# Iheckzza/FeatureMatching

Measured on AMD Instinct MI355X. Metric: image-pairs/sec at 640x480 (coarse corr + dual-softmax mutual-NN + fine window refinement), higher is better.
Workload: dtype i8 screening + f32 exact; 1 GPU; 640x480 pair, C=256 @1/8 (L=S=4800), Cf=64 @1/2, 5x5 fine window, 'peaky' descriptors; launch=hipGraph replay, concurrent_streams=4, fine_maps_layout=nchw

## Files before the change

featurematching_amd/csrc/api.hip:

```cpp
#include <math.h>
#include <stdlib.h>

#include "fm_debug.h"
#include "fm_internal.h"

namespace fm {

int g_unit_cert = 0;

int choose_splits(int N, int panels, int tiles, int target) {
  const int wg = N * panels;
#ifdef FM_TUNE_ENV
  if (const char* e = getenv("FM_TARGET_WGS")) target = atoi(e) > 0 ? atoi(e) : 256;
#endif
  int s = target / (wg > 0 ? wg : 1);
  if (s < 1) s = 1;
  const int smax = tiles / 2 > 0 ? tiles / 2 : 1;
  if (s > smax) s = smax;
  if (s > 32) s = 32;
  return s;
}

static int choose_screen_chunks(int N, int Lp, int nunits, int* units_per_chunk, bool alone) {
  const long nrb = (long)N * (Lp / 32);
// ... 10 lines not shown
  C = padded_channels(C);
  w.N = N; w.L = L; w.S = S; w.C = C; w.slots = slots;
  w.Lp = round_up(L, kPanelRows);
  w.Sp = round_up(S, kTileCols);
  w.panels = w.Lp / kPanelRows;
  w.tiles = w.Sp / kTileCols;
  w.splits = choose_splits(N, w.panels, w.tiles);
  {
    int target = N * w.panels >= kMaxPassSlots ? 10 * kMaxPassSlots : (alone ? kMaxPassSlots : kMaxPassTarget);
    if (target == kMaxPassTarget && w.tiles / choose_splits(N, w.panels, w.tiles, kMaxPassTarget) >= 32) target = kMaxPassSlots;
    w.splits0 = choose_splits(N, w.panels, w.tiles, target);
    w.top2 = N * w.panels < kMaxPassSlots && w.tiles / choose_splits(N, w.panels, w.tiles, kMaxPassTarget) < 32;
  }
#ifdef FM_TUNE_ENV
  if (const char* e = getenv("FM_TARGET_WGS0")) w.splits0 = choose_splits(N, w.panels, w.tiles, atoi(e) > 0 ? atoi(e) : kMaxPassTarget);
#endif
  w.splits_s = choose_screen_chunks(N, w.Lp, w.Sp / 32, &w.units_s, alone);
  const size_t rows = (size_t)N * w.Lp, cols = (size_t)N * w.Sp;
  const size_t nblk = (rows * slots + 255) / 256;
  size_t o = 0;
  auto take = [&](auto& r, size_t count) { r.at = o; o = align256(o + r.bytes(count)); };
  auto since = [&](size_t at) { return Span{at, o - at}; };
  take(w.cand.count, rows);
  take(w.ccand.count, cols);
  take(w.cand_b.count, rows);
  take(w.ccand_b.count, cols);
  take(w.dense_cnt, N);
  w.counters[0] = since(w.cand.count.at);
  take(w.cell0, rows);
  take(w.cell1, cols);
  take(w.ties0, kTieCap + 1);
  take(w.ties1, kTieCap + 1);
  w.reassign[0] = since(w.cell0.at);
  take(w.rowmax_u, rows);
  take(w.colmax_u, cols);
  take(w.blocktot, nblk);
  w.reassign[1] = since(w.blocktot.at);
  take(w.scalars, 1);
  w.reassign[2] = Span{w.scalars.at, sizeof(Scalars::flags)};
  w.counters[1] = Span{w.scalars.at, sizeof(Scalars)};
  w.prep_zero = since(w.cand.count.at);
  take(w.q0, rows * C); take(w.q1, cols * C);
  take(w.sigimg, (size_t)N * 2);
  take(w.imgstat, (size_t)N * 8);
  take(w.l1_0, rows); take(w.l1_1, cols);
  take(w.bstat0, rows / 32); take(w.bstat1, cols / 32);
  take(w.emarg, N);
  take(w.nmr, rows); take(w.nmc, cols);
  take(w.umax, rows / 32 * (cols / N / 32));
  take(w.cand.idx, rows * slots); take(w.cand.x, rows * slots);
  take(w.ccand.idx, cols * slots); take(w.ccand.x, cols * slots);
  take(w.thr_r, rows); take(w.thr_c, cols);
  take(w.wmaxb, rows / 32); take(w.cmaxu, cols / 32);
  take(w.tmin_r, rows / 32); take(w.tmin_c, cols / 32);
  take(w.umax2, rows / 32 * (cols / N / 32));
  take(w.upos, rows / 32 * (cols / N / 32));
  w.common_total = o;
  take(w.hi0, rows * C); take(w.lo0, rows * C);
  take(w.hi1, cols * C); take(w.lo1, cols * C);
  take(w.f16inv, N);
  take(w.rowB, rows * w.splits); take(w.colB, cols * w.panels);
  take(w.rsum, rows); take(w.csum, cols);
  take(w.nmr2, rows); take(w.nmc2, cols);
  take(w.cand_b.idx, rows * slots); take(w.cand_b.x, rows * slots);
  take(w.ccand_b.idx, cols * slots); take(w.ccand_b.x, cols * slots);
  w.total = o;
  return w;
}

}

using namespace fm;

extern "C" int fm_version(void) { return FM_VERSION; }

extern "C" const char* fm_strerror(int s) {
  switch (s) {
    case FM_OK: return "ok";
    case FM_E_NULL: return "required pointer is NULL";
    case FM_E_SHAPE: return "inconsistent or non-positive shape";
    case FM_E_UNSUPPORTED: return "unsupported configuration (C % 4 == 0 and C <= 256, Cf = 64, W in {5,7}, thr in (0,1))";
    case FM_E_WORKSPACE: return "workspace too small or not 256-byte aligned";
    case FM_E_CAPACITY: return "more matches than the output capacity";
    case FM_E_CANDIDATES: return "a coarse row or column exceeded its candidate slots (FM_MODE_EXACT_SCREENING, then more cand_slots)";
    case FM_E_RANGE: return "descriptor not finite or |x| >= 32768, or similarities of several thousand (screening margin >= 2^60)";
    case FM_E_DENSE: return "flat similarity in a sample: call again with FM_MODE_DENSE";
    case FM_E_INTERNAL: return "assignment kernel: bounded wait for predecessor workgroups ran out; call again";
    case FM_E_STEP: return "int8 screening step too small for a descriptor outside the sampled rows: call again with FM_MODE_EXACT_STEP";
    default: return s > 0 ? hipGetErrorString((hipError_t)s) : "unknown fmatch status";
  }
}

extern "C" int fm_default_cand_slots(float thr) {
  if (!(thr > 0.f)) return 64;
  int need = (int)ceilf(1.0f / thr) + 3;
  int s = 8;
  while (s < need && s < 64) s <<= 1;
  return s;
}

static float inv_ct_of(int C, float temperature) { return 1.0f / ((float)C * temperature); }

static bool valid_slots(int s) { return s >= 4 && s <= 64 && (s & (s - 1)) == 0; }

constexpr int kKnownModes = FM_MODE_DENSE | FM_MODE_EXACT_SCREENING | FM_MODE_NO_CELL_MAPS | FM_MODE_EXACT_STEP | FM_MODE_STATS |
                            FM_MODE_FLAT | FM_MODE_ALONE;

// ... 56 lines not shown
  return FM_OK;
}

extern "C" int fm_coarse_workspace_bytes(int N, int L, int S, int C, int cand_slots, size_t* bytes) {
  return fm_coarse_workspace_bytes_mode(N, L, S, C, cand_slots, FM_MODE_DENSE | FM_MODE_EXACT_SCREENING, 1, bytes);
}

extern "C" int fm_debug_coarse_layout(int N, int L, int S, int C, int cand_slots, int64_t* out, int n_out) {
  if (!out) return FM_E_NULL;
  if (n_out < 40) return FM_E_SHAPE;
  CoarseWs w;
  if (const int bad = checked_layout(true, N, L, S, C, cand_slots, &w)) return bad;
  const auto at = [](const auto& r) { return (int64_t)r.at; };
  const int64_t v[41] = {w.N, w.L, w.S, w.C, w.Lp, w.Sp, w.panels, w.tiles, w.splits, w.slots,
                         at(w.cand.count), at(w.ccand.count), at(w.scalars), at(w.blocktot), at(w.hi0), at(w.lo0),
                         at(w.hi1), at(w.lo1), at(w.q0), at(w.q1), at(w.sigimg), at(w.l1_0), at(w.nmr), at(w.nmr),
                         at(w.rowB), at(w.colB), at(w.nmr), at(w.nmc), at(w.rsum), at(w.csum), at(w.cand.idx),
                         at(w.cand.x), at(w.ccand.idx), at(w.umax), at(w.dense_cnt), at(w.rowmax_u), at(w.colmax_u),
                         w.splits_s, w.units_s, (int64_t)w.total, (int64_t)w.common_total};
  for (int i = 0; i < 40; ++i) out[i] = v[i];
  if (n_out > 40) out[40] = v[40];
  return FM_OK;
}

template <int K>
static hipError_t clear_spans(char* base, const Span (&spans)[K], hipStream_t st) {
  for (const Span& s : spans) {
    const hipError_t e = hipMemsetAsync(base + s.at, 0, s.bytes, st);
    if (e != hipSuccess) return e;
  }
  return hipSuccess;
}

static int coarse_match_impl(const CoarseCall& c, const MapCopyJob* job, bool resume) {
  if (!c.feat0 || !c.feat1 || !c.workspace || !c.d_count) return FM_E_NULL;
  if (c.in_dtype != FM_F32 && c.in_dtype != FM_F16 && c.in_dtype != FM_BF16) return FM_E_UNSUPPORTED;
  if (c.cap > 0 && (!c.b_ids || !c.i_ids || !c.j_ids || !c.mkpts0_c || !c.mkpts1_c || !c.mconf)) return FM_E_NULL;
  if (c.cap < 0 || c.L != c.h0c * c.w0c || c.S != c.h1c * c.w1c) return FM_E_SHAPE;
  if (const int bad = check_coarse_shape(c.N, c.L, c.S, c.C, c.cand_slots)) return bad;
  if (!(c.thr > 0.f) || !(c.thr < 1.f) || !(c.temperature > 0.f)) return FM_E_UNSUPPORTED;
  if (c.mode & ~kKnownModes) return FM_E_UNSUPPORTED;
  const CoarsePlan p = plan_coarse(c.mode, c.conf_matrix != nullptr, c.cand_slots);
  const CoarseWs w = coarse_layout(c.N, c.L, c.S, c.C, c.cand_slots, p.alone);
  if (c.workspace_bytes < p.workspace_bytes(w) || ((uintptr_t)c.workspace & 255)) return FM_E_WORKSPACE;
  char* base = (char*)c.workspace;
  hipStream_t st = (hipStream_t)c.stream;
  const float inv_ct = inv_ct_of(c.C, c.temperature);
  const float thr_list = fminf(c.thr, p.list_cap);
#define FM_TRY(call) do { const hipError_t e_ = (call); if (e_ != hipSuccess) return (int)e_; } while (0)
  if (!resume) {
    FM_TRY(launch_prep(c.feat0, c.feat1, c.in_dtype, c.C, w, base, p.exact_step, p.flat, st));
    FM_TRY(launch_max_i8(w, base, unit_cert_on(w, !p.dense), st));
    if (p.flat) FM_TRY(launch_stab(w, base, inv_ct, c.thr, p.allow_dead, st));
    else FM_TRY(launch_screen(c.feat0, c.feat1, c.in_dtype, c.C, w, base, inv_ct, c.thr, p.dense, p.allow_dead, st));
  } else {
    FM_TRY(clear_spans(base, w.reassign, st));
  }
  if (p.prep_f16) FM_TRY(launch_prep_f16(c.feat0, c.feat1, c.in_dtype, c.C, w, base, p.f16_force, st));
  if (p.dense) FM_TRY(launch_dense(w, base, inv_ct, thr_list, st));
  if (p.reduce) FM_TRY(launch_reduce(w, base, inv_ct, st));
  if (p.rescreen) FM_TRY(launch_dense(w, base, inv_ct, thr_list, st, nullptr, 1));
  if (p.exact_lists) FM_TRY(launch_exact_lists(w, base, inv_ct, c.feat0, c.feat1, c.in_dtype, c.C, st));
  if (p.conf) {
    FM_TRY(launch_dense(w, base, inv_ct, c.thr, st, c.conf_matrix));
    FM_TRY(launch_conf_patch(w, base, inv_ct, c.conf_matrix, st));
  }
#undef FM_TRY
  return (int)launch_select(w, base, c, inv_ct, p.select(), job);
}

extern "C" int fm_coarse_match(const float* feat0, const float* feat1, int N, int L, int S, int C, int h0c, int w0c,
                               int h1c, int w1c, float temperature, float thr, int border_rm, float scale_px,
                               const float* scale0, const float* scale1, void* workspace, size_t workspace_bytes,
                               int cand_slots, int mode, int64_t* b_ids, int64_t* i_ids, int64_t* j_ids,
                               float* mkpts0_c, float* mkpts1_c, float* mconf, int cap, int32_t* d_count,
                               float* conf_matrix, void* stream) {
  const CoarseCall c{feat0, feat1, FM_F32, N, L, S, C, h0c, w0c, h1c, w1c, temperature, thr, border_rm, scale_px, scale0, scale1,
                     workspace, workspace_bytes, cand_slots, mode, b_ids, i_ids, j_ids, mkpts0_c, mkpts1_c, mconf, cap,
                     d_count, conf_matrix, stream};
  return coarse_match_impl(c, nullptr, false);
}

extern "C" int fm_coarse_match_dtype(const void* feat0, const void* feat1, int in_dtype, int N, int L, int S, int C,
                                     int h0c, int w0c, int h1c, int w1c, float temperature, float thr, int border_rm,
                                     float scale_px, const float* scale0, const float* scale1, void* workspace,
                                     size_t workspace_bytes, int cand_slots, int mode, int64_t* b_ids,
                                     int64_t* i_ids, int64_t* j_ids, float* mkpts0_c, float* mkpts1_c, float* mconf,
                                     int cap, int32_t* d_count, float* conf_matrix, void* stream) {
  const CoarseCall c{feat0, feat1, in_dtype, N, L, S, C, h0c, w0c, h1c, w1c, temperature, thr, border_rm, scale_px, scale0,
                     scale1, workspace, workspace_bytes, cand_slots, mode, b_ids, i_ids, j_ids, mkpts0_c, mkpts1_c, mconf, cap,
                     d_count, conf_matrix, stream};
  return coarse_match_impl(c, nullptr, false);
}

extern "C" int fm_coarse_match_maps(const void* feat0, const void* feat1, int in_dtype, int N, int L, int S, int C,
                                    int h0c, int w0c, int h1c, int w1c, float temperature, float thr, int border_rm,
                                    float scale_px, const float* scale0, const float* scale1, void* workspace,
                                    size_t workspace_bytes, int cand_slots, int mode, int64_t* b_ids,
                                    int64_t* i_ids, int64_t* j_ids, float* mkpts0_c, float* mkpts1_c, float* mconf,
                                    int cap, int32_t* d_count, float* conf_matrix, const float* feat_f1, int Nf, int Cf,
                                    int Hf1, int Wf1, void* scratch1, void* stream) {
  if (!feat_f1 || !scratch1) return FM_E_NULL;
  if (Nf <= 0 || Hf1 <= 0 || Wf1 <= 0) return FM_E_SHAPE;
  if (Cf != 64) return FM_E_UNSUPPORTED;
  if (((uintptr_t)scratch1 & 15) || ((uintptr_t)feat_f1 & 15)) return FM_E_WORKSPACE;
  const MapCopyJob job{feat_f1, (float*)scratch1, Nf, Hf1, Wf1};
  const CoarseCall c{feat0, feat1, in_dtype, N, L, S, C, h0c, w0c, h1c, w1c, temperature, thr, border_rm, scale_px, scale0,
// ... 75 lines not shown
  }
  *m_out = m;
  if (info_out) *info_out = info;
  if (hint_io && (st == FM_OK || st == FM_E_CAPACITY)) {
    int learnt = cur & kAutoDataModes;
    if (full_stats) learnt &= ~FM_MODE_EXACT_SCREENING | (mode & FM_MODE_EXACT_SCREENING);
    if ((learnt & FM_MODE_DENSE) && !full_stats) {
      if (info & FM_DEV_ALL_DENSE) learnt |= FM_MODE_FLAT; else learnt &= ~FM_MODE_FLAT;
    }
    *hint_io = learnt | (slots != slots_start ? slots << 8 : 0) | (slots << 16) | (attempts << 24);
  }
  return st;
}

extern "C" int fm_coarse_cell_maps(void* workspace, int N, int L, int S, int C, int cand_slots, int32_t** cell0,
                                   int* pitch0, int32_t** ties0, int32_t** cell1, int* pitch1, int32_t** ties1) {
  CoarseWs w;
  if (const int bad = checked_layout(workspace && cell0 && cell1 && pitch0 && pitch1 && ties0 && ties1, N, L, S, C,
                                     cand_slots, &w))
    return bad;
  *cell0 = w.cell0.in(workspace); *pitch0 = w.Lp; *ties0 = w.ties0.in(workspace);
  *cell1 = w.cell1.in(workspace); *pitch1 = w.Sp; *ties1 = w.ties1.in(workspace);
  return FM_OK;
}

extern "C" int fm_coarse_softmax_stats(void* workspace, int N, int L, int S, int C, int cand_slots, const float** nm_r,
                                       const float** sum_r, int* pitch_r, const float** nm_c, const float** sum_c,
                                       int* pitch_c) {
  CoarseWs w;
  if (const int bad = checked_layout(workspace && nm_r && sum_r && pitch_r && nm_c && sum_c && pitch_c, N, L, S, C,
                                     cand_slots, &w))
    return bad;
  *nm_r = w.nmr.in(workspace); *sum_r = w.rsum.in(workspace); *pitch_r = w.Lp;
  *nm_c = w.nmc.in(workspace); *sum_c = w.csum.in(workspace); *pitch_c = w.Sp;
  return FM_OK;
}

extern "C" int fm_debug_launch_corr(void* workspace, int N, int L, int S, int C, int cand_slots, float temperature,
                                    float thr, int mode, void* stream) {
  CoarseWs w;
  if (const int bad = checked_layout(workspace, N, L, S, C, cand_slots, &w)) return bad;
  if (mode < 0 || mode > 2) return FM_E_UNSUPPORTED;
  hipStream_t st = (hipStream_t)stream;
  if (mode == 0) return (int)launch_max_i8(w, (char*)workspace, unit_cert_on(w), st);
  if (mode == 1) return (int)launch_dense(w, (char*)workspace, inv_ct_of(C, temperature), thr, st);
  return (int)launch_dense(w, (char*)workspace, inv_ct_of(C, temperature), thr, st, nullptr, 1);
}

extern "C" int fm_debug_launch_screen(void* workspace, const float* feat0, const float* feat1, int N, int L, int S,
                                          int C, int cand_slots, float temperature, float thr, void* stream) {
  CoarseWs w;
  if (const int bad = checked_layout(workspace && feat0 && feat1, N, L, S, C, cand_slots, &w)) return bad;
  return (int)launch_screen(feat0, feat1, FM_F32, C, w, (char*)workspace, inv_ct_of(C, temperature), thr, 1, 1,
                                (hipStream_t)stream);
}

extern "C" int fm_debug_launch_prep(void* workspace, const float* feat0, const float* feat1, int N, int L, int S, int C,
                                    int cand_slots, void* stream) {
  CoarseWs w;
  if (const int bad = checked_layout(workspace && feat0 && feat1, N, L, S, C, cand_slots, &w)) return bad;
  return (int)launch_prep(feat0, feat1, FM_F32, C, w, (char*)workspace, 0, 0, (hipStream_t)stream);
}

extern "C" int fm_debug_launch_prep_f16(void* workspace, const float* feat0, const float* feat1, int N, int L, int S,
                                        int C, int cand_slots, int force, void* stream) {
  CoarseWs w;
  if (const int bad = checked_layout(workspace && feat0 && feat1, N, L, S, C, cand_slots, &w)) return bad;
  return (int)launch_prep_f16(feat0, feat1, FM_F32, C, w, (char*)workspace, force, (hipStream_t)stream);
}

extern "C" int fm_debug_launch_flat(void* workspace, const float* feat0, const float* feat1, int N, int L, int S, int C,
                                    int cand_slots, float temperature, float thr, int which, void* stream) {
  CoarseWs w;
  if (const int bad = checked_layout(workspace && feat0 && feat1, N, L, S, C, cand_slots, &w)) return bad;
  if (which < 0 || which > 1) return FM_E_UNSUPPORTED;
  if (which == 0) return (int)launch_prep(feat0, feat1, FM_F32, C, w, (char*)workspace, 0, 1, (hipStream_t)stream);
  return (int)launch_stab(w, (char*)workspace, inv_ct_of(C, temperature), thr, 1, (hipStream_t)stream);
}

extern "C" int fm_debug_reset_counters(void* workspace, int N, int L, int S, int C, int cand_slots, void* stream) {
  CoarseWs w;
  if (const int bad = checked_layout(workspace, N, L, S, C, cand_slots, &w)) return bad;
  return (int)clear_spans((char*)workspace, w.counters, (hipStream_t)stream);
}

extern "C" int fm_debug_unit_cert(int mode) {
  const int prev = g_unit_cert;
  if (mode >= 0 && mode <= 2) g_unit_cert = mode;
  return prev;
}

extern "C" int fm_debug_unit_cert_layout(int N, int L, int S, int C, int cand_slots, int64_t* out, int n_out) {
  if (!out) return FM_E_NULL;
  if (n_out < 9) return FM_E_SHAPE;
  CoarseWs w;
  if (const int bad = checked_layout(true, N, L, S, C, cand_slots, &w)) return bad;
  const int64_t v[9] = {(int64_t)w.umax.at, (int64_t)w.umax2.at, (int64_t)w.upos.at, (int64_t)w.thr_r.at, (int64_t)w.thr_c.at,
                        (int64_t)w.tmin_r.at, (int64_t)w.tmin_c.at, (int64_t)(w.scalars.at + offsetof(Scalars, cert_units)), w.top2};
  for (int i = 0; i < 9; ++i) out[i] = v[i];
  return FM_OK;
}

extern "C" int fm_read_count(const int32_t* d_count, int cap, int32_t* m_out, void* stream) {
  return fm_read_count_info(d_count, cap, m_out, nullptr, stream);
}

extern "C" int fm_read_count_info(const int32_t* d_count, int cap, int32_t* m_out, int32_t* info_out, void* stream) {
  if (!d_count || !m_out) return FM_E_NULL;
  int32_t h[2] = {0, 0};
  hipStream_t st = (hipStream_t)stream;
  hipError_t e = hipMemcpyAsync(h, d_count, sizeof(h), hipMemcpyDeviceToHost, st);
  if (e != hipSuccess) return (int)e;
  e = hipStreamSynchronize(st);
  if (e != hipSuccess) return (int)e;
  *m_out = h[0];
  if (info_out) *info_out = h[1];
  if (h[1] & FM_DEV_INTERNAL) return FM_E_INTERNAL;
  if (h[1] & FM_DEV_RANGE) return FM_E_RANGE;
  if (h[1] & FM_DEV_STEP) return FM_E_STEP;
  if (h[1] & FM_DEV_DENSE) return FM_E_DENSE;
  if (h[1] & FM_DEV_CANDIDATES) return FM_E_CANDIDATES;
  if (h[1] & FM_DEV_CAPACITY) return FM_E_CAPACITY;
  if (h[0] > cap) return FM_E_CAPACITY;
  return FM_OK;
}
```

featurematching_amd/csrc/coarse_screen.hip:

```cpp
#include <stdlib.h>
#include <string.h>

#include <type_traits>

#include "fm_device.h"
#include "fm_wave_device.h"

namespace fm {

constexpr int kMaxExact = 24;

struct ScreenArgs {
  const signed char* q0; const signed char* q1;
  const void* src0; const void* src1; int c_in, in_dtype;
  const unsigned* rowmax_u; const unsigned* colmax_u;
  const float* sigimg;
  const float* imgstat;
  const float* l1_0; const float* l1_1;
  const float4* bstat0; const float4* bstat1;
  const float* umax;
  float* nmr; float* nmc; float* emarg;
  int* dense_cnt; Scalars* scal;
  int* rcount; int* rlist_j; float* rlist_x;
  int* ccount; int* clist_i; float* clist_x;
  int L, S, Lp, Sp, slots, dense_enabled;
  int allow_dead;
  float k, lt, inv_ct, cpad;
};

__device__ __forceinline__ int sig_threshold(float nm, float emu, float inv_kss) {
  const float t = floorf((-kSkipLog2 - emu - nm) * inv_kss) - 1.f;
  return (int)fminf(fmaxf(t, -1.0e9f), 1.0e9f);
}

__global__ __launch_bounds__(256) void k_stab(ScreenArgs a, float* f16inv) {
  const int side = blockIdx.z, b = blockIdx.y;
  const int len = side ? a.S : a.L, lenp = side ? a.Sp : a.Lp;
  const int idx = blockIdx.x * 256 + threadIdx.x;
  const float sig0 = a.sigimg[b * 2], sig1 = a.sigimg[b * 2 + 1];
  const float* ist = a.imgstat + (long)b * 8;
  const float l1A_max = ist[0], clipA = ist[1], infA = ist[2], l1B_max = ist[3], clipB = ist[4], infB = ist[5];
  const float ss = sig0 * sig1;
  if (blockIdx.x == 0 && side == 0 && threadIdx.x == 0) {
    const float emarg = margin_log2(q8_margin_raw(sig0, l1A_max, clipA, sig1, l1B_max, clipB, a.cpad), a.inv_ct);
    a.emarg[b] = emarg;
    const bool clipped = clipA > 0.f || clipB > 0.f;
    const float sc0 = f16_plane_scale(127.f * sig0), sc1 = f16_plane_scale(127.f * sig1);
    f16inv[b] = (1.0f / sc0) * (1.0f / sc1);
    if (!(l1A_max < INFINITY) || !(l1B_max < INFINITY)) atomicOr(&a.scal->flags, (unsigned)FM_DEV_RANGE);
    else if (!(emarg < 60.f)) atomicOr(&a.scal->flags, (unsigned)(clipped ? FM_DEV_STEP : FM_DEV_RANGE));
    else if (!(infA * sc0 < 65504.f) || !(infB * sc1 < 65504.f)) atomicOr(&a.scal->flags, (unsigned)FM_DEV_STEP);
    a.dense_cnt[b] = 1;
    a.scal->dense_units = 1;
  }
  if (idx >= lenp) return;
  const long g = (long)b * lenp + idx;
  float nm = -INFINITY;
  if (idx < len) {
    const float ln2 = 0.69314718f;
    const float l1 = (side ? a.l1_1 : a.l1_0)[g];
    const unsigned mx = (side ? a.colmax_u : a.rowmax_u)[g];
    const bool dead = a.allow_dead && 2.002f * l1 * (side ? infA : infB) * a.inv_ct + 1e-3f <
                                          (a.lt + __builtin_log2f((float)(side ? a.L : a.S))) * ln2;
    const float mraw = side ? q8_margin_raw(sig0, l1A_max, clipA, sig1, l1, clipB, a.cpad)
                            : q8_margin_raw(sig0, l1, clipA, sig1, l1B_max, clipB, a.cpad);
    nm = dead ? -INFINITY : neg_stabiliser_log2(ss * q_decode(mx), mraw, a.inv_ct);
  }
  (side ? a.nmc : a.nmr)[g] = nm;
}

struct RowsExtra {
  int* thr_r; int* thr_c; float* wmaxb; float* cmaxu;
  int* tmin_r; int* tmin_c;
  const int* umax2; const int* upos;
  int look;
  int count_cert;
  int nchunks, chunk_units, items;
};

__global__ __launch_bounds__(256) void k_thresh(ScreenArgs a, RowsExtra x) {
  const int side = blockIdx.z, b = blockIdx.y;
  const int len = side ? a.S : a.L, lenp = side ? a.Sp : a.Lp;
  const int idx = blockIdx.x * 256 + threadIdx.x;
  const int lane = threadIdx.x & 63;
  const float sig0 = a.sigimg[b * 2], sig1 = a.sigimg[b * 2 + 1];
  const float* ist = a.imgstat + (long)b * 8;
  const float l1A_max = ist[0], clipA = ist[1], infA = ist[2], l1B_max = ist[3], clipB = ist[4], infB = ist[5];
  const float ss = sig0 * sig1;
  const float kss = a.k * ss;
  const bool screen_ok = kss > 1e-30f && kss < 1e30f;
  const float inv_kss = screen_ok ? 1.0f / kss : 0.f;
  if (blockIdx.x == 0 && side == 0 && threadIdx.x == 0) {
    const float emarg = margin_log2(q8_margin_raw(sig0, l1A_max, clipA, sig1, l1B_max, clipB, a.cpad), a.inv_ct);
    a.emarg[b] = emarg;
    const bool clipped = clipA > 0.f || clipB > 0.f;
    const float emarg0 = margin_log2(q8_margin_raw(sig0, l1A_max, 0.f, sig1, l1B_max, 0.f, a.cpad), a.inv_ct);
    if (!(l1A_max < INFINITY) || !(l1B_max < INFINITY)) atomicOr(&a.scal->flags, (unsigned)FM_DEV_RANGE);
    else if (!(emarg < 60.f)) atomicOr(&a.scal->flags, (unsigned)(clipped ? FM_DEV_STEP : FM_DEV_RANGE));
    else if (clipped && emarg > 2.0f * emarg0 + 1.0f) atomicOr(&a.scal->flags, (unsigned)FM_DEV_STEP);
  }
  if (idx >= lenp) return;
  const long g = (long)b * lenp + idx;
  const int blk = idx >> 5;
  const int nblk = lenp / 32;
  float nm = -INFINITY;
  float emu = 0.f;
  if (idx < len) {
    const float ln2 = 0.69314718f;
    const float l1 = (side ? a.l1_1 : a.l1_0)[g];
    const unsigned mx = (side ? a.colmax_u : a.rowmax_u)[g];
    const float bl1 = (side ? a.bstat1 : a.bstat0)[(long)b * nblk + blk].x;
    const bool dead = a.allow_dead && 2.002f * l1 * (side ? infA : infB) * a.inv_ct + 1e-3f <
                                          (a.lt + __builtin_log2f((float)(side ? a.L : a.S))) * ln2;
    const float mraw = side ? q8_margin_raw(sig0, l1A_max, clipA, sig1, l1, clipB, a.cpad)
                            : q8_margin_raw(sig0, l1, clipA, sig1, l1B_max, clipB, a.cpad);
    nm = dead ? -INFINITY : neg_stabiliser_log2(ss * q_decode(mx), mraw, a.inv_ct);
    emu = margin_log2(side ? q8_margin_raw(sig0, l1A_max, clipA, sig1, bl1, clipB, a.cpad)
                           : q8_margin_raw(sig0, bl1, clipA, sig1, l1B_max, clipB, a.cpad), a.inv_ct);
  }
  (side ? a.nmc : a.nmr)[g] = nm;
  const int thr = idx < len ? sig_threshold(nm, emu, inv_kss) : 0x3fffffff;
  (side ? x.thr_c : x.thr_r)[g] = thr;
  const float bm = half_all<OpMax>(nm);
  const int tm = half_all<OpMin>(thr);
  if ((lane & 31) == 0) {
    (side ? x.cmaxu : x.wmaxb)[(long)b * nblk + blk] = bm;
    (side ? x.tmin_c : x.tmin_r)[(long)b * nblk + blk] = tm;
  }
}

template <int C>
__global__ __launch_bounds__(256, 3) void k_screen_rows(ScreenArgs a, RowsExtra x) {
  constexpr int KS8 = C / 32;
  constexpr int LIST = 256;
  const int tid = threadIdx.x;
  const int lane = tid & 63;
  const int wv = __builtin_amdgcn_readfirstlane(tid >> 6);
  const int r = lane & 31, h = lane >> 5;
  __shared__ int s_list[4][LIST];

  const int nrb = a.Lp / 32, nunits = a.Sp / 32;
  const int item = xcd_contiguous(blockIdx.x, gridDim.x) * 4 + wv;
  if (item >= x.items) return;
  const int per_sample = nrb * x.nchunks;
  const int b = item / per_sample;
  int kk = item - b * per_sample;
  const int chunk = kk / nrb;
  const int rb = kk - chunk * nrb;
  const int wrow0 = rb * 32;
  if (wrow0 >= a.L) return;
  const int u0 = chunk * x.chunk_units;
  const int U = min(x.chunk_units, nunits - u0);

  const float sig0 = a.sigimg[b * 2], sig1 = a.sigimg[b * 2 + 1];
  const float* ist = a.imgstat + (long)b * 8;
  const float clipA = ist[1], clipB = ist[4];
  const float bl1A = a.bstat0[(long)b * nrb + rb].x;
  const float wmax = x.wmaxb[(long)b * nrb + rb];
  const int ul_c = min(lane, U - 1);
  const float um = a.umax[((long)b * nrb + rb) * nunits + u0 + ul_c];
  const float cm = x.cmaxu[(long)b * nunits + u0 + ul_c];
  const float bl1B = a.bstat1[(long)b * nunits + u0 + ul_c].x;
  const bool look = x.look && ist[6] != 0.f;
  const int um2 = x.umax2[((long)b * nrb + rb) * nunits + u0 + ul_c];
  const int upos = x.upos[((long)b * nrb + rb) * nunits + u0 + ul_c];
  const int tmin = min(x.tmin_r[(long)b * nrb + rb], x.tmin_c[(long)b * nunits + u0 + ul_c]);
  int trr[16];
  {
    const int* tp = x.thr_r + (long)b * a.Lp + wrow0 + 4 * h;
#pragma unroll
    for (int q = 0; q < 4; ++q) {
      const int4 t4 = *reinterpret_cast<const int4*>(tp + 8 * q);
      trr[4 * q] = t4.x; trr[4 * q + 1] = t4.y; trr[4 * q + 2] = t4.z; trr[4 * q + 3] = t4.w;
    }
  }
  v4i aq[KS8];
  {
    const signed char* src = a.q0 + (((long)b * a.Lp + wrow0) / 32 * KS8 * 64 + lane) * 16;
#pragma unroll
    for (int ks = 0; ks < KS8; ++ks) aq[ks] = *reinterpret_cast<const v4i*>(src + ks * 1024);
  }
  const float ss = sig0 * sig1;
  const float kss = a.k * ss;
  const bool screen_ok = kss > 1e-30f && kss < 1e30f;

  unsigned long long live;
  {
    const float emu = margin_log2(q8_margin_raw(sig0, bl1A, clipA, sig1, bl1B, clipB, a.cpad), a.inv_ct);
    const float top = __builtin_fmaf(um, kss, emu);
    const bool hot = lane < U && (!screen_ok || !((top + wmax < -kSkipLog2) && (top + cm < -kSkipLog2)));
    live = __ballot(hot);
  }
  const unsigned long long cert = look ? (live & __ballot(um2 <= tmin)) : 0ull;
  live &= ~cert;
  const bool flat = !screen_ok || a.dense_cnt[b] != 0;
  int nd_units = flat ? 1 : 0;
  int nlist = 0;
#ifdef FM_ABL_ROWS
  if (FM_ABL_ROWS & 1) live = 0;
#endif
  int cert_thr = 0x3fffffff, cert_key = 0;
  if (!flat && ((cert >> lane) & 1)) {
    const int g = upos & 15, lw = (upos >> 4) & 63;
    const int rl = (g & 3) + 8 * (g >> 2) + 4 * (lw >> 5), cl = lw & 31;
    cert_thr = min(x.thr_r[(long)b * a.Lp + wrow0 + rl], x.thr_c[(long)b * a.Sp + (u0 + lane) * 32 + cl]);
    cert_key = (lane << 10) | (rl << 5) | cl;
  }
  if (x.count_cert && cert && lane == 0) atomicAdd(&a.scal->cert_units, __builtin_popcountll(cert));
  if (!flat && live) {
    const bool row_edge = (wrow0 + 32 > a.L);
    const signed char* q1b = a.q1 + ((long)b * nunits + u0) * KS8 * 1024 + lane * 16;
    const int* tcb = x.thr_c + (long)b * a.Sp + u0 * 32 + r;
    auto load_unit = [&](int ul, v4i (&bq)[KS8], int& tcl) {
      const signed char* src = q1b + (long)ul * KS8 * 1024;
#pragma unroll
      for (int ks = 0; ks < KS8; ++ks) bq[ks] = *reinterpret_cast<const v4i*>(src + ks * 1024);
      tcl = tcb[ul * 32];
    };
    auto screen_unit = [&](int ul, const v4i (&bq)[KS8], int tcl) {
      const int ucol0 = (u0 + ul) * 32;
      v16i acc;
#pragma unroll
      for (int g = 0; g < 16; ++g) acc[g] = 0;
#pragma unroll
      for (int ks = 0; ks < KS8; ++ks) acc = __builtin_amdgcn_mfma_i32_32x32x32_i8(aq[ks], bq[ks], acc, 0, 0, 0);
      if (row_edge || ucol0 + 32 > a.S) {
        const bool cok = ucol0 + r < a.S;
#pragma unroll
        for (int g = 0; g < 16; ++g)
          if (!cok || wrow0 + (g & 3) + 8 * (g >> 2) + 4 * h >= a.L) acc[g] = kQMasked;
      }
      unsigned bm = 0;
#pragma unroll
      for (int g = 0; g < 16; ++g) bm |= (acc[g] > min(trr[g], tcl)) ? (1u << g) : 0u;
      unsigned long long hitl = __ballot(bm != 0);
      if (!hitl) return;
      int cnt = 0;
#pragma unroll
      for (int g = 0; g < 16; ++g) cnt += __builtin_popcountll(__ballot((bm >> g) & 1u));
      if (cnt > kMaxExact || nlist + cnt > LIST) { ++nd_units; return; }
      while (hitl) {
        const int l = __builtin_ctzll(hitl);
        hitl &= hitl - 1;
        unsigned bits = (unsigned)__builtin_amdgcn_readlane((int)bm, l);
        while (bits) {
          const int g = __builtin_ctz(bits);
          bits &= bits - 1;
          const int rl = (g & 3) + 8 * (g >> 2) + 4 * (l >> 5);
          if (lane == 0) s_list[wv][nlist] = (ul << 10) | (rl << 5) | (l & 31);
          ++nlist;
        }
      }
    };
    v4i bA[KS8], bB[KS8];
    int tcA = 0, tcB = 0;
    unsigned long long mask = live;
    int ulA = __builtin_ctzll(mask), ulB = -1;
    mask &= mask - 1;
    load_unit(ulA, bA, tcA);
    while (true) {
      ulB = -1;
      if (mask) { ulB = __builtin_ctzll(mask); mask &= mask - 1; load_unit(ulB, bB, tcB); }
      screen_unit(ulA, bA, tcA);
      if (ulB < 0 || nd_units) break;
      ulA = -1;
      if (mask) { ulA = __builtin_ctzll(mask); mask &= mask - 1; load_unit(ulA, bA, tcA); }
      screen_unit(ulB, bB, tcB);
      if (ulA < 0 || nd_units) break;
    }
  }
  if (!flat && cert && !nd_units) {
    const unsigned long long hits = __ballot((int)um > cert_thr);
    const int nh = __builtin_popcountll(hits);
    if (nlist + nh > LIST) ++nd_units;
    else {
      if ((hits >> lane) & 1) s_list[wv][nlist + __builtin_popcountll(hits & ((1ull << lane) - 1ull))] = cert_key;
      nlist += nh;
    }
  }
  if (nd_units) nlist = 0;

  int overflow = 0;
#ifdef FM_ABL_ROWS
  if (FM_ABL_ROWS & 2) nlist = 0;
#endif
  {
    constexpr int NPASS = 4;
    const int sub = lane >> 4, l16 = lane & 15;
    const int vpr = a.c_in >> 2;
    for (int e0 = 0; e0 < nlist; e0 += 4 * NPASS) {
      int myres = 0;
      float my_nmr = 0.f, my_nmc = 0.f;
      if (lane < 4 * NPASS && e0 + lane < nlist) {
        const int ky = s_list[wv][e0 + lane];
        const int row = wrow0 + ((ky >> 5) & 31), col = (u0 + ((ky >> 10) & 63)) * 32 + (ky & 31);
        const int pr = atomicAdd(&a.rcount[(long)b * a.Lp + row], 1);
        const int pc = atomicAdd(&a.ccount[(long)b * a.Sp + col], 1);
        my_nmr = a.nmr[(long)b * a.Lp + row];
        my_nmc = a.nmc[(long)b * a.Sp + col];
        myres = min(pr, 0xffff) | (min(pc, 0xffff) << 16);
      }
      int key[NPASS];
      float xs[NPASS];
#pragma unroll
      for (int h2 = 0; h2 < NPASS; h2 += 2) {
        float4 av[2][4], bv[2][4];
#pragma unroll
        for (int pp = 0; pp < 2; ++pp) {
          const int p = h2 + pp;
          const int idx = e0 + 4 * p + sub;
          key[p] = s_list[wv][min(idx, nlist - 1)];
          const int row = wrow0 + ((key[p] >> 5) & 31), col = (u0 + ((key[p] >> 10) & 63)) * 32 + (key[p] & 31);
          const long ro = ((long)b * a.L + row) * a.c_in, co = ((long)b * a.S + col) * a.c_in;
#pragma unroll
          for (int q = 0; q < 4; ++q) {
            const int v4 = l16 + 16 * q;
            const bool in = v4 < vpr;
            const int vc = in ? v4 : 0;
            float4 ta, tb;
            if (a.in_dtype == FM_F32) {
              ta = reinterpret_cast<const float4*>((const float*)a.src0 + ro)[vc];
              tb = reinterpret_cast<const float4*>((const float*)a.src1 + co)[vc];
            } else {
              ta = half4_to_float4(reinterpret_cast<const uint2*>((const unsigned short*)a.src0 + ro)[vc], a.in_dtype);
              tb = half4_to_float4(reinterpret_cast<const uint2*>((const unsigned short*)a.src1 + co)[vc], a.in_dtype);
// ... 17 lines not shown
        if (e0 + 4 * (h2 + 2) >= nlist) break;
      }
#pragma unroll
      for (int p = 0; p < NPASS; ++p) {
        const int idx = e0 + 4 * p + sub;
        if (e0 + 4 * p >= nlist) break;
        const int pos = __shfl(myres, 4 * p + sub);
        const float nmr_e = __shfl(my_nmr, 4 * p + sub), nmc_e = __shfl(my_nmc, 4 * p + sub);
        if (l16 == 0 && idx < nlist) {
          const int row = wrow0 + ((key[p] >> 5) & 31), col = (u0 + ((key[p] >> 10) & 63)) * 32 + (key[p] & 31);
          const float rr = __builtin_fmaf(xs[p], a.k, nmr_e);
          const float cc = __builtin_fmaf(xs[p], a.k, nmc_e);
          const int pr = pos & 0xffff, pc = (pos >> 16) & 0xffff;
          const long grow = (long)b * a.Lp + row, gcol = (long)b * a.Sp + col;
          if (pr < a.slots) { a.rlist_j[grow * a.slots + pr] = col; a.rlist_x[grow * a.slots + pr] = rr > -kSkipLog2 ? xs[p] : -INFINITY; }
          else overflow = 1;
          if (pc < a.slots) { a.clist_i[gcol * a.slots + pc] = row; a.clist_x[gcol * a.slots + pc] = cc > -kSkipLog2 ? xs[p] : -INFINITY; }
          else overflow = 1;
        }
      }
    }
  }
  nd_units += __builtin_popcountll(__ballot(overflow != 0));
  if (nd_units && lane == 0) {
    a.dense_cnt[b] = 1;
    a.scal->dense_units = 1;
    if (!a.dense_enabled) atomicOr(&a.scal->flags, (unsigned)FM_DEV_DENSE);
  }
}

static void fill_screen_stats(ScreenArgs& a, const CoarseWs& w, char* base, float inv_ct, float thr, int allow_dead) {
  a.rowmax_u = w.rowmax_u.in(base); a.colmax_u = w.colmax_u.in(base);
  a.sigimg = w.sigimg.in(base); a.imgstat = w.imgstat.in(base);
  a.l1_0 = w.l1_0.in(base); a.l1_1 = w.l1_1.in(base);
  a.bstat0 = w.bstat0.in(base); a.bstat1 = w.bstat1.in(base);
  a.umax = w.umax.in(base);
  a.nmr = w.nmr.in(base); a.nmc = w.nmc.in(base); a.emarg = w.emarg.in(base);
  a.dense_cnt = w.dense_cnt.in(base); a.scal = w.scalars.in(base);
  a.L = w.L; a.S = w.S; a.Lp = w.Lp; a.Sp = w.Sp;
  a.slots = w.slots; a.allow_dead = allow_dead;
  a.k = inv_ct * kLog2e; a.lt = log2f(thr); a.inv_ct = inv_ct; a.cpad = (float)w.C;
}

hipError_t launch_stab(const CoarseWs& w, char* base, float inv_ct, float thr, int allow_dead, hipStream_t st) {
  ScreenArgs a;
  memset(&a, 0, sizeof(a));
  fill_screen_stats(a, w, base, inv_ct, thr, allow_dead);
  const int lenp = w.Lp > w.Sp ? w.Lp : w.Sp;
  hipLaunchKernelGGL(k_stab, dim3((lenp + 255) / 256, w.N, 2), dim3(256), 0, st, a, w.f16inv.in(base));
  return hipGetLastError();
}

hipError_t launch_screen(const void* feat0, const void* feat1, int in_dtype, int c_in, const CoarseWs& w, char* base,
                         float inv_ct, float thr, int dense_enabled, int allow_dead, hipStream_t st) {
  ScreenArgs a;
  memset(&a, 0, sizeof(a));
  fill_screen_stats(a, w, base, inv_ct, thr, allow_dead);
  a.in_dtype = in_dtype;
  a.q0 = w.q0.in(base); a.q1 = w.q1.in(base);
  a.src0 = feat0; a.src1 = feat1; a.c_in = c_in;
  a.rcount = w.cand.count.in(base); a.rlist_j = w.cand.idx.in(base); a.rlist_x = w.cand.x.in(base);
  a.ccount = w.ccand.count.in(base); a.clist_i = w.ccand.idx.in(base); a.clist_x = w.ccand.x.in(base);
  a.dense_enabled = dense_enabled;
  RowsExtra x;
  x.thr_r = w.thr_r.in(base); x.thr_c = w.thr_c.in(base);
  x.wmaxb = w.wmaxb.in(base); x.cmaxu = w.cmaxu.in(base);
  x.tmin_r = w.tmin_r.in(base); x.tmin_c = w.tmin_c.in(base);
  x.umax2 = w.umax2.in(base); x.upos = w.upos.in(base);
  x.look = g_unit_cert != 1;
  x.count_cert = g_unit_cert == 2;
  x.chunk_units = w.units_s;
  x.nchunks = w.splits_s;
#ifdef FM_TUNE_ENV
  if (const char* ev = getenv("FM_ROWS_CHUNK")) { x.chunk_units = atoi(ev); x.nchunks = (w.Sp / 32 + x.chunk_units - 1) / x.chunk_units; }
#endif
  x.items = (int)((long)w.N * (w.Lp / 32) * x.nchunks);
  const int lenp = w.Lp > w.Sp ? w.Lp : w.Sp;
  hipLaunchKernelGGL(k_thresh, dim3((lenp + 255) / 256, w.N, 2), dim3(256), 0, st, a, x);
  const int blocks_r = (x.items + 3) / 4;
  return with_padded_channels(w.C, [&](auto cc) {
    hipLaunchKernelGGL(k_screen_rows<cc.value>, dim3(blocks_r), dim3(256), 0, st, a, x);
    return hipGetLastError();
  });
}

}
```

featurematching_amd/csrc/fm_internal.h:

```cpp
#pragma once
#include <hip/hip_runtime.h>
#include <stddef.h>
#include <stdint.h>

#include <type_traits>

#include "fmatch.h"

namespace fm {

constexpr int kPanelRows = 256;
constexpr int kTieCap = 1023;
constexpr int kTileCols = 64;
constexpr float kLog2e = 1.4426950408889634f;
constexpr float kSkipLog2 = 32.f;
constexpr unsigned FM_INT_SCREEN_OVERFLOW = 16u;
constexpr unsigned FM_INT_LOOKBACK_TIMEOUT = 64u;
constexpr int kPrepSampleRows = 32;
constexpr float kPrepHeadroom = 1.5f;

inline int round_up(int x, int m) { return (x + m - 1) / m * m; }
inline int padded_channels(int c) { return c <= 64 ? 64 : (c <= 128 ? 128 : 256); }
inline bool valid_channels(int c) { return c >= 4 && c <= 256 && c % 4 == 0; }
inline size_t align256(size_t x) { return (x + 255) & ~size_t(255); }

struct Span { size_t at, bytes; };
template <typename T>
inline T* span_ptr(void* base, const Span& s) { return reinterpret_cast<T*>(static_cast<char*>(base) + s.at); }
template <typename T>
struct Region {
  size_t at;
  T* in(void* base) const { return reinterpret_cast<T*>(static_cast<char*>(base) + at); }
  static size_t bytes(size_t count) { return count * sizeof(T); }
};
struct CandList { Region<int> count, idx; Region<float> x; };

template <int V> using int_c = std::integral_constant<int, V>;
template <typename F>
inline bool with_window(int W, F&& f) {
  if (W == 5) f(int_c<5>{});
  else if (W == 7) f(int_c<7>{});
  else return false;
  return true;
}

inline bool crop_shape_ok(int N, int Hf, int Wf, int stride, int m_max) {
  return N > 0 && Hf > 0 && Wf > 0 && stride > 0 && m_max >= 0;
}

struct Scalars {
  unsigned flags;
  int dense_units;
  int cert_units;
};

struct CoarseWs {
  int N, L, S, C, Lp, Sp, panels, tiles, splits, slots;
  int splits0;
  int splits_s, units_s;
  int top2;
  Span prep_zero;
  Span reassign[3];
  Span counters[2];
  CandList cand, ccand;
  CandList cand_b, ccand_b;
  Region<int> dense_cnt;
  Region<Scalars> scalars;
  Region<int> cell0, cell1;
  Region<int> ties0, ties1;
  Region<unsigned> rowmax_u, colmax_u;
  Region<int> blocktot;
  Region<signed char> q0, q1;
  Region<float> sigimg;
  Region<float> imgstat;
  Region<float> l1_0, l1_1;
  Region<float4> bstat0, bstat1;
  Region<float> emarg;
  Region<float> nmr, nmc;
  Region<float> umax;
  Region<int> thr_r, thr_c;
  Region<float> wmaxb, cmaxu;
  Region<int> tmin_r, tmin_c;
  Region<int> umax2, upos;
  size_t common_total;
  Region<_Float16> hi0, lo0, hi1, lo1;
  Region<float> f16inv;
  Region<float> rowB, colB;
  Region<float> rsum, csum;
  Region<float> nmr2, nmc2;
  size_t total;
};

int choose_splits(int N, int panels, int tiles, int target = 256);
CoarseWs coarse_layout(int N, int L, int S, int C, int slots, bool alone = false);

extern int g_unit_cert;
inline bool unit_cert_on(const CoarseWs& w, bool common_path = true) {
  return g_unit_cert == 2 || (g_unit_cert == 0 && w.top2 != 0 && common_path);
}

struct CoarseCall {
  const void *feat0, *feat1; int in_dtype;
  int N, L, S, C, h0c, w0c, h1c, w1c;
  float temperature, thr; int border_rm; float scale_px; const float *scale0, *scale1;
  void* workspace; size_t workspace_bytes;
  int cand_slots, mode;
  int64_t *b_ids, *i_ids, *j_ids; float *mkpts0_c, *mkpts1_c, *mconf; int cap; int32_t* d_count; float* conf_matrix;
  void* stream;
};

hipError_t launch_prep(const void* feat0, const void* feat1, int in_dtype, int c_in, const CoarseWs& w, char* base,
                       int exact_step, int planes, hipStream_t st);
hipError_t launch_stab(const CoarseWs& w, char* base, float inv_ct, float thr, int allow_dead, hipStream_t st);
hipError_t launch_prep_f16(const void* feat0, const void* feat1, int in_dtype, int c_in, const CoarseWs& w, char* base,
                           int force, hipStream_t st);
hipError_t launch_max_i8(const CoarseWs& w, char* base, bool top2, hipStream_t st);
hipError_t launch_dense(const CoarseWs& w, char* base, float inv_ct, float thr, hipStream_t st, float* conf = nullptr,
                        int rescreen = 0);
hipError_t launch_reduce(const CoarseWs& w, char* base, float inv_ct, hipStream_t st);
struct MapCopyJob {
  const float* src; float* dst; int N, Hf, Wf;
};
struct SelectFlags { bool exact, dense, cell_maps, sums_ready; };
hipError_t launch_select(const CoarseWs& w, char* base, const CoarseCall& c, float inv_ct, SelectFlags flags,
                         const MapCopyJob* job = nullptr);
hipError_t launch_conf_patch(const CoarseWs& w, char* base, float inv_ct, float* conf, hipStream_t st);
hipError_t launch_exact_lists(const CoarseWs& w, char* base, float inv_ct, const void* feat0, const void* feat1, int in_dtype,
                              int c_in, hipStream_t st);
hipError_t launch_screen(const void* feat0, const void* feat1, int in_dtype, int c_in, const CoarseWs& w, char* base,
                             float inv_ct, float thr, int dense_enabled, int allow_dead, hipStream_t st);

struct DsmBwdWs { Span v, u, sums, part; size_t total; };
inline DsmBwdWs dsm_bwd_layout(int N, int L, int S, int C) {
  DsmBwdWs w;
  w.v = {0, (size_t)N * L * 4};
  w.u = {w.v.bytes, (size_t)N * S * 4};
  w.sums = {0, w.v.bytes + w.u.bytes};
  w.part = {align256(w.sums.bytes), (size_t)4 * N * (size_t)(L > S ? L : S) * C * 4};
  w.total = w.part.at + w.part.bytes;
  return w;
}
struct DsmStats {
  const float *ofs_r, *sum_r; int pitch_r;
  const float *ofs_c, *sum_c; int pitch_c;
};
struct DsmProblem {
  const float *feat0, *feat1;
  int N, L, S, C;
  float k2, inv_ct;
  float *v, *u, *part;
};
int dsm_carve(const float* feat0, const float* feat1, int N, int L, int S, int C, float temperature, const DsmStats& s,
              void* workspace, size_t workspace_bytes, DsmProblem* p);
int dsm_begin(const float* feat0, const float* feat1, int N, int L, int S, int C, float temperature, const DsmStats& s,
              void* workspace, size_t workspace_bytes, hipStream_t st, DsmProblem* p);
int dsm_zsplit(int N, int R);
struct DsmSide { DsmProblem p; DsmStats s; };
inline DsmSide dsm_side(const DsmProblem& p, const DsmStats& s, int side) {
  if (!side) return {p, s};
  return {{p.feat1, p.feat0, p.N, p.S, p.L, p.C, p.k2, p.inv_ct, p.u, p.v, p.part},
          {s.ofs_c, s.sum_c, s.pitch_c, s.ofs_r, s.sum_r, s.pitch_r}};
}
inline dim3 dsm_sweep_grid(const DsmSide& o) { return dim3((o.p.L + 31) / 32, o.p.N, dsm_zsplit(o.p.N, o.p.L)); }
template <typename F>
inline hipError_t with_padded_channels(int C, F&& f) {
  const int Cp = padded_channels(C);
  return Cp == 64 ? f(int_c<64>{}) : Cp == 128 ? f(int_c<128>{}) : f(int_c<256>{});
}
hipError_t launch_sweep_combine(const DsmSide& o, int Z, const float* d_loss, float* d_out, hipStream_t st);
hipError_t launch_dsm_uv(const int64_t* b_ids, const int64_t* i_ids, const int64_t* j_ids, const float* gc, int K, int L, int S,
                         float* v, float* u, hipStream_t st);
hipError_t launch_dsm_entries(const DsmProblem& p, const int64_t* b_ids, const int64_t* i_ids, const int64_t* j_ids,
                              const float* gc, int K, float* d_feat0, float* d_feat1, hipStream_t st);

template <typename K>
inline hipError_t ensure_dynamic_lds(K kernel, int bytes, unsigned long long* done_mask) {
  int dev = 0;
  hipError_t e = hipGetDevice(&dev);
  if (e != hipSuccess) return e;
  const unsigned long long bit = 1ull << (dev & 63);
  if (__atomic_load_n(done_mask, __ATOMIC_ACQUIRE) & bit) return hipSuccess;
  e = hipFuncSetAttribute(reinterpret_cast<const void*>(kernel), hipFuncAttributeMaxDynamicSharedMemorySize, bytes);
  if (e == hipSuccess) __atomic_fetch_or(done_mask, bit, __ATOMIC_RELEASE);
// ... 5 lines not shown
```

Measured before the change: 20600 image-pairs/s.

## Add per-block threshold max to resolve certified units without per-unit gathers

The threshold kernel now also records the per-block maximum of the thresholds, stored next to the minimum. The screen kernel uses it to sort certified units into sure hits (unit max above both block maxima) and ambiguous ones. Only ambiguous units gather per-element row and column thresholds. The screen kernel is also templated on whether certification is enabled, so the non-cert variant drops those loads, and in the cert variant the sweep-state loads are deferred until after classification. This adds workspace, an extra max reduction in k_thresh and two template instantiations.

```diff
diff --git a/featurematching_amd/csrc/api.hip b/featurematching_amd/csrc/api.hip
--- a/featurematching_amd/csrc/api.hip
+++ b/featurematching_amd/csrc/api.hip
@@ -86,7 +86,8 @@
   take(w.ccand.idx, cols * slots); take(w.ccand.x, cols * slots);
   take(w.thr_r, rows); take(w.thr_c, cols);
   take(w.wmaxb, rows / 32); take(w.cmaxu, cols / 32);
-  take(w.tmin_r, rows / 32); take(w.tmin_c, cols / 32);
+  take(w.tmin_r, 2 * (rows / 32)); take(w.tmin_c, 2 * (cols / 32));
+  w.tmax_r.at = w.tmin_r.at + w.tmin_r.bytes(rows / 32); w.tmax_c.at = w.tmin_c.at + w.tmin_c.bytes(cols / 32);
   take(w.umax2, rows / 32 * (cols / N / 32));
   take(w.upos, rows / 32 * (cols / N / 32));
   w.common_total = o;
@@ -249,7 +250,8 @@
     FM_TRY(launch_prep(c.feat0, c.feat1, c.in_dtype, c.C, w, base, p.exact_step, p.flat, st));
     FM_TRY(launch_max_i8(w, base, unit_cert_on(w, !p.dense), st));
     if (p.flat) FM_TRY(launch_stab(w, base, inv_ct, c.thr, p.allow_dead, st));
-    else FM_TRY(launch_screen(c.feat0, c.feat1, c.in_dtype, c.C, w, base, inv_ct, c.thr, p.dense, p.allow_dead, st));
+    else FM_TRY(launch_screen(c.feat0, c.feat1, c.in_dtype, c.C, w, base, inv_ct, c.thr, p.dense, p.allow_dead,
+                              unit_cert_on(w, !p.dense), st));
   } else {
     FM_TRY(clear_spans(base, w.reassign, st));
   }
@@ -431,7 +433,7 @@
   CoarseWs w;
   if (const int bad = checked_layout(workspace && feat0 && feat1, N, L, S, C, cand_slots, &w)) return bad;
   return (int)launch_screen(feat0, feat1, FM_F32, C, w, (char*)workspace, inv_ct_of(C, temperature), thr, 1, 1,
-                                (hipStream_t)stream);
+                                unit_cert_on(w), (hipStream_t)stream);
 }
 
 extern "C" int fm_debug_launch_prep(void* workspace, const float* feat0, const float* feat1, int N, int L, int S, int C,
@@ -474,9 +476,11 @@
   if (n_out < 9) return FM_E_SHAPE;
   CoarseWs w;
   if (const int bad = checked_layout(true, N, L, S, C, cand_slots, &w)) return bad;
-  const int64_t v[9] = {(int64_t)w.umax.at, (int64_t)w.umax2.at, (int64_t)w.upos.at, (int64_t)w.thr_r.at, (int64_t)w.thr_c.at,
-                        (int64_t)w.tmin_r.at, (int64_t)w.tmin_c.at, (int64_t)(w.scalars.at + offsetof(Scalars, cert_units)), w.top2};
-  for (int i = 0; i < 9; ++i) out[i] = v[i];
+  const int64_t v[13] = {(int64_t)w.umax.at, (int64_t)w.umax2.at, (int64_t)w.upos.at, (int64_t)w.thr_r.at, (int64_t)w.thr_c.at,
+                         (int64_t)w.tmin_r.at, (int64_t)w.tmin_c.at, (int64_t)(w.scalars.at + offsetof(Scalars, cert_units)), w.top2,
+                         (int64_t)w.tmax_r.at, (int64_t)w.tmax_c.at, (int64_t)(w.scalars.at + offsetof(Scalars, range_units)),
+                         (int64_t)(w.scalars.at + offsetof(Scalars, gather_units))};
+  for (int i = 0; i < (n_out < 13 ? 9 : 13); ++i) out[i] = v[i];
   return FM_OK;
 }
 
diff --git a/featurematching_amd/csrc/coarse_screen.hip b/featurematching_amd/csrc/coarse_screen.hip
--- a/featurematching_amd/csrc/coarse_screen.hip
+++ b/featurematching_amd/csrc/coarse_screen.hip
@@ -76,6 +76,7 @@
   int look;
   int count_cert;
   int nchunks, chunk_units, items;
+  int nsamp;
 };
 
 __global__ __launch_bounds__(256) void k_thresh(ScreenArgs a, RowsExtra x) {
@@ -122,14 +123,17 @@
   const int thr = idx < len ? sig_threshold(nm, emu, inv_kss) : 0x3fffffff;
   (side ? x.thr_c : x.thr_r)[g] = thr;
   const float bm = half_all<OpMax>(nm);
+  if ((lane & 31) == 0) (side ? x.cmaxu : x.wmaxb)[(long)b * nblk + blk] = bm;
+  if (!x.look) return;
   const int tm = half_all<OpMin>(thr);
+  const int tx = half_all<OpMax>(idx < len ? thr : -0x7fffffff);
   if ((lane & 31) == 0) {
-    (side ? x.cmaxu : x.wmaxb)[(long)b * nblk + blk] = bm;
     (side ? x.tmin_c : x.tmin_r)[(long)b * nblk + blk] = tm;
-  }
-}
-
-template <int C>
+    (side ? x.tmin_c : x.tmin_r)[((long)gridDim.y + b) * nblk + blk] = tx == -0x7fffffff ? 0x3fffffff : tx;
+  }
+}
+
+template <int C, bool CERT>
 __global__ __launch_bounds__(256, 3) void k_screen_rows(ScreenArgs a, RowsExtra x) {
   constexpr int KS8 = C / 32;
   constexpr int LIST = 256;
@@ -154,32 +158,38 @@
 
   const float sig0 = a.sigimg[b * 2], sig1 = a.sigimg[b * 2 + 1];
   const float* ist = a.imgstat + (long)b * 8;
-  const float clipA = ist[1], clipB = ist[4];
+  const float clipA = ist[1], clipB = ist[4], top2_written = ist[6];
+  const int dense_flagged = a.dense_cnt[b];
   const float bl1A = a.bstat0[(long)b * nrb + rb].x;
   const float wmax = x.wmaxb[(long)b * nrb + rb];
   const int ul_c = min(lane, U - 1);
   const float um = a.umax[((long)b * nrb + rb) * nunits + u0 + ul_c];
   const float cm = x.cmaxu[(long)b * nunits + u0 + ul_c];
   const float bl1B = a.bstat1[(long)b * nunits + u0 + ul_c].x;
-  const bool look = x.look && ist[6] != 0.f;
-  const int um2 = x.umax2[((long)b * nrb + rb) * nunits + u0 + ul_c];
-  const int upos = x.upos[((long)b * nrb + rb) * nunits + u0 + ul_c];
-  const int tmin = min(x.tmin_r[(long)b * nrb + rb], x.tmin_c[(long)b * nunits + u0 + ul_c]);
+  const bool look = CERT && top2_written != 0.f;
+  int um2 = 0, upos = 0, tmin = 0, thi = 0;
+  if constexpr (CERT) {
+    const long nsamp = x.nsamp;
+    um2 = x.umax2[((long)b * nrb + rb) * nunits + u0 + ul_c];
+    upos = x.upos[((long)b * nrb + rb) * nunits + u0 + ul_c];
+    tmin = min(x.tmin_r[(long)b * nrb + rb], x.tmin_c[(long)b * nunits + u0 + ul_c]);
+    thi = min(x.tmin_r[(nsamp + b) * nrb + rb], x.tmin_c[(nsamp + b) * nunits + u0 + ul_c]);
+  }
   int trr[16];
-  {
+  v4i aq[KS8];
+  auto load_sweep_state = [&]() {
     const int* tp = x.thr_r + (long)b * a.Lp + wrow0 + 4 * h;
 #pragma unroll
     for (int q = 0; q < 4; ++q) {
       const int4 t4 = *reinterpret_cast<const int4*>(tp + 8 * q);
       trr[4 * q] = t4.x; trr[4 * q + 1] = t4.y; trr[4 * q + 2] = t4.z; trr[4 * q + 3] = t4.w;
     }
-  }
-  v4i aq[KS8];
-  {
     const signed char* src = a.q0 + (((long)b * a.Lp + wrow0) / 32 * KS8 * 64 + lane) * 16;
 #pragma unroll
     for (int ks = 0; ks < KS8; ++ks) aq[ks] = *reinterpret_cast<const v4i*>(src + ks * 1024);
-  }
+  };
+  constexpr bool sweep_early = !CERT;
+  if (sweep_early) load_sweep_state();
   const float ss = sig0 * sig1;
   const float kss = a.k * ss;
   const bool screen_ok = kss > 1e-30f && kss < 1e30f;
@@ -191,32 +201,62 @@
     const bool hot = lane < U && (!screen_ok || !((top + wmax < -kSkipLog2) && (top + cm < -kSkipLog2)));
     live = __ballot(hot);
   }
-  const unsigned long long cert = look ? (live & __ballot(um2 <= tmin)) : 0ull;
+  const unsigned long long cert = live & __ballot(look & (um2 <= tmin));
   live &= ~cert;
-  const bool flat = !screen_ok || a.dense_cnt[b] != 0;
+  const bool flat = !screen_ok | (dense_flagged != 0);
   int nd_units = flat ? 1 : 0;
   int nlist = 0;
 #ifdef FM_ABL_ROWS
   if (FM_ABL_ROWS & 1) live = 0;
 #endif
-  int cert_thr = 0x3fffffff, cert_key = 0;
-  if (!flat && ((cert >> lane) & 1)) {
-    const int g = upos & 15, lw = (upos >> 4) & 63;
-    const int rl = (g & 3) + 8 * (g >> 2) + 4 * (lw >> 5), cl = lw & 31;
-    cert_thr = min(x.thr_r[(long)b * a.Lp + wrow0 + rl], x.thr_c[(long)b * a.Sp + (u0 + lane) * 32 + cl]);
-    cert_key = (lane << 10) | (rl << 5) | cl;
-  }
+  const bool sweeps = !flat && live != 0;
+  const signed char* q1b = a.q1 + ((long)b * nunits + u0) * KS8 * 1024 + lane * 16;
+  const int* tcb = x.thr_c + (long)b * a.Sp + u0 * 32 + r;
+  auto load_unit = [&](int ul, v4i (&bq)[KS8], int& tcl) {
+    const signed char* src = q1b + (long)ul * KS8 * 1024;
+#pragma unroll
+    for (int ks = 0; ks < KS8; ++ks) bq[ks] = *reinterpret_cast<const v4i*>(src + ks * 1024);
+    tcl = tcb[ul * 32];
+  };
+  v4i bA[KS8], bB[KS8];
+  int tcA = 0, tcB = 0;
+  unsigned long long mask = live;
+  int ulA = -1, ulB = -1;
+  int cert_key = 0, cert_tr = 0x3fffffff, cert_tc = 0x3fffffff;
+  bool sure = false, amb = false;
   if (x.count_cert && cert && lane == 0) atomicAdd(&a.scal->cert_units, __builtin_popcountll(cert));
-  if (!flat && live) {
+  auto classify = [&]() {
+    if (flat || !cert) return;
+    {
+      const bool mine = (cert >> lane) & 1;
+      const int umi = (int)um;
+      const int g = upos & 15, lw = (upos >> 4) & 63;
+      const int rl = (g & 3) + 8 * (g >> 2) + 4 * (lw >> 5), cl = lw & 31;
+      cert_key = (lane << 10) | (rl << 5) | cl;
+      sure = mine && umi > thi;
+      amb = mine && !sure && umi > tmin;
+      if (__any(amb)) {
+        cert_tr = x.thr_r[(long)b * a.Lp + wrow0 + rl];
+        cert_tc = x.thr_c[(long)b * a.Sp + (u0 + ul_c) * 32 + cl];
+      }
+      if (x.count_cert) {
+        const int ns = __builtin_popcountll(__ballot(sure)), na = __builtin_popcountll(__ballot(amb));
+        if (lane == 0 && ns) atomicAdd(&a.scal->range_units, ns);
+        if (lane == 0 && na) atomicAdd(&a.scal->gather_units, na);
+      }
+    }
+  };
+  if (sweeps) {
+    classify();
+    if (!sweep_early) load_sweep_state();
+    ulA = __builtin_ctzll(mask);
+    mask &= mask - 1;
+    load_unit(ulA, bA, tcA);
+  } else {
+    classify();
+  }
+  if (sweeps) {
     const bool row_edge = (wrow0 + 32 > a.L);
-    const signed char* q1b = a.q1 + ((long)b * nunits + u0) * KS8 * 1024 + lane * 16;
-    const int* tcb = x.thr_c + (long)b * a.Sp + u0 * 32 + r;
-    auto load_unit = [&](int ul, v4i (&bq)[KS8], int& tcl) {
-      const signed char* src = q1b + (long)ul * KS8 * 1024;
-#pragma unroll
-      for (int ks = 0; ks < KS8; ++ks) bq[ks] = *reinterpret_cast<const v4i*>(src + ks * 1024);
-      tcl = tcb[ul * 32];
-    };
     auto screen_unit = [&](int ul, const v4i (&bq)[KS8], int tcl) {
       const int ucol0 = (u0 + ul) * 32;
       v16i acc;
@@ -252,12 +292,6 @@
         }
       }
     };
-    v4i bA[KS8], bB[KS8];
-    int tcA = 0, tcB = 0;
-    unsigned long long mask = live;
-    int ulA = __builtin_ctzll(mask), ulB = -1;
-    mask &= mask - 1;
-    load_unit(ulA, bA, tcA);
     while (true) {
       ulB = -1;
       if (mask) { ulB = __builtin_ctzll(mask); mask &= mask - 1; load_unit(ulB, bB, tcB); }
@@ -270,7 +304,7 @@
     }
   }
   if (!flat && cert && !nd_units) {
-    const unsigned long long hits = __ballot((int)um > cert_thr);
+    const unsigned long long hits = __ballot(sure || (amb && (int)um > min(cert_tr, cert_tc)));
     const int nh = __builtin_popcountll(hits);
     if (nlist + nh > LIST) ++nd_units;
     else {
@@ -394,7 +428,7 @@
 }
 
 hipError_t launch_screen(const void* feat0, const void* feat1, int in_dtype, int c_in, const CoarseWs& w, char* base,
-                         float inv_ct, float thr, int dense_enabled, int allow_dead, hipStream_t st) {
+                         float inv_ct, float thr, int dense_enabled, int allow_dead, bool unit_cert, hipStream_t st) {
   ScreenArgs a;
   memset(&a, 0, sizeof(a));
   fill_screen_stats(a, w, base, inv_ct, thr, allow_dead);
@@ -409,7 +443,7 @@
   x.wmaxb = w.wmaxb.in(base); x.cmaxu = w.cmaxu.in(base);
   x.tmin_r = w.tmin_r.in(base); x.tmin_c = w.tmin_c.in(base);
   x.umax2 = w.umax2.in(base); x.upos = w.upos.in(base);
-  x.look = g_unit_cert != 1;
+  x.look = unit_cert;
   x.count_cert = g_unit_cert == 2;
   x.chunk_units = w.units_s;
   x.nchunks = w.splits_s;
@@ -417,11 +451,13 @@
   if (const char* ev = getenv("FM_ROWS_CHUNK")) { x.chunk_units = atoi(ev); x.nchunks = (w.Sp / 32 + x.chunk_units - 1) / x.chunk_units; }
 #endif
   x.items = (int)((long)w.N * (w.Lp / 32) * x.nchunks);
+  x.nsamp = w.N;
   const int lenp = w.Lp > w.Sp ? w.Lp : w.Sp;
   hipLaunchKernelGGL(k_thresh, dim3((lenp + 255) / 256, w.N, 2), dim3(256), 0, st, a, x);
   const int blocks_r = (x.items + 3) / 4;
   return with_padded_channels(w.C, [&](auto cc) {
-    hipLaunchKernelGGL(k_screen_rows<cc.value>, dim3(blocks_r), dim3(256), 0, st, a, x);
+    if (unit_cert) hipLaunchKernelGGL((k_screen_rows<cc.value, true>), dim3(blocks_r), dim3(256), 0, st, a, x);
+    else hipLaunchKernelGGL((k_screen_rows<cc.value, false>), dim3(blocks_r), dim3(256), 0, st, a, x);
     return hipGetLastError();
   });
 }
diff --git a/featurematching_amd/csrc/fm_internal.h b/featurematching_amd/csrc/fm_internal.h
--- a/featurematching_amd/csrc/fm_internal.h
+++ b/featurematching_amd/csrc/fm_internal.h
@@ -52,6 +52,9 @@
   unsigned flags;
   int dense_units;
   int cert_units;
+  int range_units;
+  int gather_units;
+  int pad[3];
 };
 
 struct CoarseWs {
@@ -81,6 +84,7 @@
   Region<int> thr_r, thr_c;
   Region<float> wmaxb, cmaxu;
   Region<int> tmin_r, tmin_c;
+  Region<int> tmax_r, tmax_c;
   Region<int> umax2, upos;
   size_t common_total;
   Region<_Float16> hi0, lo0, hi1, lo1;
@@ -128,7 +132,7 @@
 hipError_t launch_exact_lists(const CoarseWs& w, char* base, float inv_ct, const void* feat0, const void* feat1, int in_dtype,
                               int c_in, hipStream_t st);
 hipError_t launch_screen(const void* feat0, const void* feat1, int in_dtype, int c_in, const CoarseWs& w, char* base,
-                             float inv_ct, float thr, int dense_enabled, int allow_dead, hipStream_t st);
+                             float inv_ct, float thr, int dense_enabled, int allow_dead, bool unit_cert, hipStream_t st);
 
 struct DsmBwdWs { Span v, u, sums, part; size_t total; };
 inline DsmBwdWs dsm_bwd_layout(int N, int L, int S, int C) {
```

After: 20800 image-pairs/s, median of 5. Within noise of the previous version (+0.9%).
